# lucasjinreal/yolov7_d2

Hardware: AMD Instinct MI355X
Metric: images/sec training, YOLOX-s 640x640 bs=16/GPU (higher is better)
Workload: dtype bf16; 1 GPU; YOLOX-s CSPDarknet+PAFPN 640x640 bs=16/GPU: fwd + SimOTA loss + bwd + grad all-reduce + SGD(momentum) step, uint8 image batch + labels resident in HBM; global_batch=16, parallelism=dp1, hipgraph=True

## Files before the change

### yolov7_d2_amd/csrc/conv_igemm.hip

```cpp
#include <string.h>
#include <string.h>
#include "common.h"
#include "conv_igemm_kernel.h"
#include "conv1x1_stream.h"

bool c1s_try_launch(const mi_conv_desc* ds, int n, hipStream_t s, int* rc);
bool c1s_try_plan(const mi_conv_desc* ds, int n, C1Launch* l);
bool c1s_try_route(const mi_conv_desc* d);
int c1s_run_planned(const C1Launch* l, hipStream_t s);
bool c1s_try_plan_bn(const mi_conv_desc* ds, const mi_bn_job* bn, int n, C1Launch* l);
int c1s_barrier_status(unsigned* flag);
static_assert(sizeof(C1Launch) <= sizeof(((mi_conv_group*)0)->priv), "mi_conv_group.priv holds the stream launch record");
#include "conv3x3_ws.h"
bool w3_try_launch(const mi_conv_desc* ds, int n, hipStream_t s, int* rc);
bool w3_try_plan(const mi_conv_desc* ds, int n, W3Launch* l);
int w3_run_planned(const W3Launch* l, hipStream_t s);
bool w3_try_plan_bn(const mi_conv_desc* ds, const mi_bn_job* bn, int n, W3Launch* l);
int w3_barrier_status(unsigned* flag);
static_assert(sizeof(W3Launch) <= sizeof(((mi_conv_group*)0)->priv), "mi_conv_group.priv holds the 3x3 launch record");

#define MI_DECL_KC(KCv)                                                                      \
  int conv_launch_kc##KCv(const ConvK& k, int BN, int TPIX, size_t lds, hipStream_t s);       \
  int conv_group_launch_kc##KCv(const mi_conv_group* m, const ConvK* jobs, const int* starts, hipStream_t s);
MI_DECL_KC(16) MI_DECL_KC(32) MI_DECL_KC(64) MI_DECL_KC(128)
#undef MI_DECL_KC

static void choose_tile(int TPIX, int gridH, int gridW, int* TH, int* TW) {
  const int cands[] = {gridW, 64, 32, 16, 8, 4};
  long best = -1;
  int bh = 8, bw = 16;
  for (int c : cands) {
    if (c <= 0 || c > TPIX) continue;
    int tw = c;
    int th = TPIX / tw;
    if (th > gridH) th = gridH;
    if (th < 1) th = 1;
    long tiles = (long)mi_cdiv(gridH, th) * mi_cdiv(gridW, tw);
    long halo = (long)(th + 2) * (tw + 2);
    long score = tiles * 100000 + halo;
    if (best < 0 || score < best) {
      best = score;
      bh = th;
      bw = tw;
    }
  }
  *TH = bh;
  *TW = bw;
}

struct ConvCfg {
  int KC, BN, TPIX, TPS;
};

#ifdef MI_CONV_TIMELINE
static long long* g_conv_tl = nullptr;
extern "C" void mi_debug_conv_timeline(long long* dev_buf) { g_conv_tl = dev_buf; }
#endif
static int conv_fill(const mi_conv_desc* d, ConvK* k, ConvCfg* c, size_t* ldsBytes) {
  MI_REQUIRE(d->x && d->w && d->y, "conv: null pointer");
  MI_REQUIRE(d->ntaps >= 1 && d->ntaps <= MI_MAX_TAPS, "conv: ntaps %d", d->ntaps);
  MI_REQUIRE(d->K8 >= 2 && (d->K8 % 2) == 0, "conv: K8 %d must be even", d->K8);
  MI_REQUIRE(d->CoutPad % 32 == 0 && d->Cout <= d->CoutPad && d->Cout > 0, "conv: Cout %d pad %d",
             d->Cout, d->CoutPad);
  MI_REQUIRE(d->ldx % 8 == 0 && ((uintptr_t)d->x % 16) == 0, "conv: x must be 16B aligned (ldx %d)", d->ldx);
  MI_REQUIRE(d->in_stride == 1 || d->in_stride == 2, "conv: in_stride");
  MI_REQUIRE(d->out_stride == 1 || d->out_stride == 2, "conv: out_stride");
  MI_REQUIRE((long long)d->H * d->W * d->ldx < (1LL << 30), "conv: image plane too large for 32-bit offsets");
  if (!(d->flags & MI_CONV_OUT_F32))
    MI_REQUIRE((d->Cout % 4 != 0) || (d->ldy % 4 == 0 && ((uintptr_t)d->y % 8) == 0),
               "conv: bf16 y needs 8B alignment (ldy %d)", d->ldy);
  k->x = (const __bf16*)d->x;
  k->w = (const u32x4*)d->w;
  k->y = d->y;
  k->bias = d->bias;
  k->stats = d->stats_acc;
  k->nslots = (d->stats_slots >= 1 && d->stats_slots <= MI_BN_SLOTS) ? d->stats_slots : MI_BN_SLOTS;
  k->ynstride = d->y_nstride > 0 ? (long long)d->y_nstride : (long long)d->outH * d->outW * d->ldy;
  k->ldx = d->ldx; k->ldy = d->ldy; k->N = d->N; k->H = d->H; k->W = d->W;
  k->outH = d->outH; k->outW = d->outW; k->gridH = d->gridH; k->gridW = d->gridW;
  k->is = d->in_stride; k->os = d->out_stride; k->ooy = d->out_oy; k->oox = d->out_ox;
  k->K8 = d->K8; k->Cout = d->Cout; k->CoutPad = d->CoutPad; k->ntaps = d->ntaps;
  int dymin = 1 << 30, dymax = -(1 << 30), dxmin = 1 << 30, dxmax = -(1 << 30);
  for (int t = 0; t < d->ntaps; ++t) {
    k->tw[t] = d->tap_w[t];
    if (d->tap_dy[t] < dymin) dymin = d->tap_dy[t];
    if (d->tap_dy[t] > dymax) dymax = d->tap_dy[t];
    if (d->tap_dx[t] < dxmin) dxmin = d->tap_dx[t];
    if (d->tap_dx[t] > dxmax) dxmax = d->tap_dx[t];
  }
  k->flags = d->flags;
  {
    static const int noatom = getenv("MI_DEBUG_NOATOM") ? atoi(getenv("MI_DEBUG_NOATOM")) : 0;
    if (noatom) k->flags |= 1024;
  }
  MI_REQUIRE(!(d->flags & MI_CONV_RELU) || !((d->flags & (MI_CONV_ACCUM | MI_CONV_BNBWD | MI_CONV_OUT_F32 | MI_CONV_RELUMASK | MI_CONV_ADDRELU)) || d->stats_acc),
             "conv: MI_CONV_RELU is a plain forward epilogue (bf16 output, no accumulate / statistics)");
  if (d->flags & MI_CONV_BNBWD) {
    MI_REQUIRE(d->stats_acc && d->bn_y && d->bn_scale && d->bn_shift && d->bn_mean && d->bn_invstd,
               "conv: MI_CONV_BNBWD needs stats_acc and the producing layer's bn_* arrays");
    MI_REQUIRE(!(d->flags & MI_CONV_OUT_F32) && d->Cout % 8 == 0 && d->bn_ldy % 8 == 0 && ((uintptr_t)d->bn_y % 16) == 0,
               "conv: MI_CONV_BNBWD needs a bf16 output with Cout %% 8 == 0 (staged epilogue) and 16B-aligned bn_y");
    k->bn_y = (const __bf16*)d->bn_y; k->bn_scale = d->bn_scale; k->bn_shift = d->bn_shift;
    k->bn_mean = d->bn_mean; k->bn_invstd = d->bn_invstd; k->bn_ldy = d->bn_ldy; k->bn_act = d->bn_act;
  } else if (d->flags & (MI_CONV_RELUMASK | MI_CONV_ADDRELU)) {
    MI_REQUIRE((d->flags & (MI_CONV_RELUMASK | MI_CONV_ADDRELU)) != (MI_CONV_RELUMASK | MI_CONV_ADDRELU) && !d->stats_acc,
               "conv: MI_CONV_RELUMASK and MI_CONV_ADDRELU exclude each other and the forward statistics");
    MI_REQUIRE(d->bn_y && !(d->flags & MI_CONV_OUT_F32) && d->Cout % 8 == 0 && d->bn_ldy % 8 == 0 && d->bn_ldy >= d->Cout &&
               ((uintptr_t)d->bn_y % 16) == 0,
               "conv: the aux-tensor epilogue needs bn_y (16B-aligned, bn_ldy %% 8 == 0) and a bf16 output with Cout %% 8 == 0");
    k->bn_y = (const __bf16*)d->bn_y; k->bn_ldy = d->bn_ldy;
    k->bn_scale = k->bn_shift = k->bn_mean = k->bn_invstd = nullptr; k->bn_act = 0;
  } else {
    k->bn_y = nullptr; k->bn_scale = k->bn_shift = k->bn_mean = k->bn_invstd = nullptr; k->bn_ldy = 0; k->bn_act = 0;
  }
  const int Kp = d->K8 * 8;
  int BNmax = (d->CoutPad % 128 == 0) ? 128 : (d->CoutPad % 64 == 0) ? 64 : 32;
  int BN = d->BN, TPIX = 0, TH = d->TH, TW = d->TW;
  if (TH > 0 && TW > 0) TPIX = (TH * TW <= 64) ? 64 : 128;
  if (BN <= 0 || TPIX == 0) {
    const long want = 256;
    const int order[5][2] = {{128, 128}, {128, 64}, {64, 128}, {64, 64}, {64, 32}};
    int bestBN = BNmax, bestTP = TPIX ? TPIX : 128;
    for (int o = 0; o < 5; ++o) {
      const int tp = order[o][0];
      int bn = order[o][1];
      if (bn > BNmax) bn = BNmax;
      if (TPIX && tp != TPIX) continue;
      if (d->BN > 0 && bn != d->BN) continue;
      int th, tw;
      choose_tile(tp, d->gridH, d->gridW, &th, &tw);
      const long tiles = (long)d->N * mi_cdiv(d->gridH, th) * mi_cdiv(d->gridW, tw);
      bestBN = bn; bestTP = tp;
      if (tiles * (d->CoutPad / bn) >= want) break;
    }
    BN = bestBN; TPIX = bestTP;
  }
  MI_REQUIRE(BN == 32 || BN == 64 || BN == 128, "conv: BN %d", BN);
  MI_REQUIRE(d->CoutPad % BN == 0, "conv: CoutPad %d %% BN %d", d->CoutPad, BN);
  if (TH <= 0 || TW <= 0) choose_tile(TPIX, d->gridH, d->gridW, &TH, &TW);
  MI_REQUIRE(TH * TW <= TPIX && TH >= 1 && TW >= 1, "conv: tile %dx%d", TH, TW);
  k->TH = TH; k->TW = TW;
  k->tilesY = mi_cdiv(d->gridH, TH); k->tilesX = mi_cdiv(d->gridW, TW);
  k->dymin = dymin; k->dxmin = dxmin;
  const int haloH = (TH - 1) * d->in_stride + (dymax - dymin) + 1;
  k->haloW = (TW - 1) * d->in_stride + (dxmax - dxmin) + 1;
  k->npixh = haloH * k->haloW;
  for (int t = 0; t < d->ntaps; ++t) k->toff[t] = (d->tap_dy[t] - dymin) * k->haloW + (d->tap_dx[t] - dxmin);
  k->nco = d->CoutPad / BN;
  const long nblocks = (long)d->N * k->tilesY * k->tilesX * k->nco;
  int KC = d->KC, tps = d->TPS;
  auto lds_need = [&](int kc, int tp) {
    const size_t xb = (size_t)mi_cdiv(k->npixh, 64 / (kc / 8)) * 1024;
    const size_t wb = (size_t)tp * (kc / 8) * BN * 16;
    const int nch = Kp / kc, nst = nch * (d->ntaps / tp);
    return xb * (nch > 1 ? 2 : 1) + wb * (nst > 1 ? 2 : 1);
  };
  if (KC <= 0 || tps <= 0) {
    static const int maxkc = getenv("MI_CONV_MAXKC") ? atoi(getenv("MI_CONV_MAXKC")) : 128;
    static const int cap2 = getenv("MI_CONV_LDSCAP") ? atoi(getenv("MI_CONV_LDSCAP")) : 80;
    static const int cap1 = getenv("MI_CONV_LDSCAP1") ? atoi(getenv("MI_CONV_LDSCAP1")) : 160;
    static const double cS = getenv("MI_CONV_S") ? atof(getenv("MI_CONV_S")) : 0.25;
    static const double cT = getenv("MI_CONV_T") ? atof(getenv("MI_CONV_T")) : 0.3;
    static const int useocc = getenv("MI_CONV_OCC") ? atoi(getenv("MI_CONV_OCC")) : 1;
    const size_t cap = (size_t)(nblocks > 256 ? cap2 : cap1) * 1024;
    double bestCost = -1.0;
    int bk = 16, bt = 1;
    size_t bestLds = 0;
    const double vocc = BN == 32 ? 8.0 : (BN == 64 ? (TPIX == 128 ? 4.0 : 8.0) : (TPIX == 128 ? 3.0 : 5.0));
    const double gocc = nblocks > 256 ? nblocks / 256.0 : 1.0;
    const int kcs[4] = {128, 64, 32, 16};
    for (int ci = 0; ci < 4; ++ci) {
      const int kc = kcs[ci];
      if (Kp % kc != 0 || (d->KC > 0 && kc != d->KC) || (d->KC <= 0 && kc > maxkc)) continue;
      for (int tp = d->ntaps; tp >= 1; --tp) {
        if (d->ntaps % tp != 0 || (d->TPS > 0 && tp != d->TPS)) continue;
        const size_t need = lds_need(kc, tp);
        if (need > cap && !(kc == 16 && tp == 1)) continue;
        double occ = (double)((160 * 1024) / (need > 20480 ? need : 20480));
        if (occ < 1.0) occ = 1.0;
        if (occ > vocc) occ = vocc;
        if (occ > gocc) occ = gocc;
        if (!useocc) occ = 1.0;
        const double steps = (double)(Kp / kc) * (d->ntaps / tp), iters = (double)(Kp / kc) * d->ntaps;
        const double cost = (steps * cS + iters * cT) / occ;
        if (bestCost < 0 || cost < bestCost * 0.999 || (cost <= bestCost * 1.001 && need < bestLds)) {
          bestCost = cost; bk = kc; bt = tp; bestLds = need;
        }
      }
    }
    KC = bk; tps = bt;
  }
  MI_REQUIRE((KC == 16 || KC == 32 || KC == 64 || KC == 128) && Kp % KC == 0, "conv: KC %d for K %d", KC, Kp);
  MI_REQUIRE(tps >= 1 && d->ntaps % tps == 0, "conv: TPS %d for %d taps", tps, d->ntaps);
  const int RPI = 64 / (KC / 8);
  k->nqx = mi_cdiv(k->npixh, RPI);
  k->xbytes = k->nqx * 1024;
  MI_REQUIRE((long)k->nqx * RPI * k->haloW < (1 << 20) && k->nqx * RPI < 4096, "conv: halo too large for the row decode");
  k->mTW = ((1u << 20) + TW - 1) / TW;
  k->mHW = ((1u << 20) + k->haloW - 1) / k->haloW;
  const int nch = Kp / KC, nst = nch * (d->ntaps / tps);
  k->tps = tps;
  k->xstride = nch > 1 ? k->xbytes : 0;
  k->wstride = nst > 1 ? tps * (KC / 8) * BN * 16 : 0;
  c->KC = KC; c->BN = BN; c->TPIX = TPIX; c->TPS = tps;
  {
    static const int xm = getenv("MI_CONV_XMAP") ? atoi(getenv("MI_CONV_XMAP")) : 2;
    const bool on = xm >= 3 || (xm == 2 && (k->nco > 1 || d->ntaps > 1)) || (xm == 1 && k->nco > 1);
    k->xmap = (on && nblocks % 8 == 0) ? (int)(nblocks / 8) : 0;
#ifdef MI_CONV_TIMELINE
    k->tl = g_conv_tl;
#endif
  }
  *ldsBytes = lds_need(KC, tps);
  const size_t stage = (size_t)TPIX * (BN * 2 + 16);
  const size_t red = (size_t)16 * BN * 8;
  if (*ldsBytes < stage) *ldsBytes = stage;
  if (*ldsBytes < red) *ldsBytes = red;
  if (*ldsBytes < 4 * BN * 8) *ldsBytes = 4 * BN * 8;
  MI_REQUIRE(*ldsBytes <= 160 * 1024, "conv: LDS %zu too large", *ldsBytes);
  return MI_OK;
}

extern "C" int mi_conv2d_route(const mi_conv_desc* d) {
  MI_REQUIRE(d, "conv2d_route: null");
  if (c1s_try_route(d)) return 1;
  W3Launch wl;
  if (w3_try_plan(d, 1, &wl)) return 2;
  return d->xf ? -1 : 0;
}

extern "C" int mi_conv2d_plan(mi_conv_desc* d) {
  ConvK k;
  ConvCfg c;
  size_t lds;
  int rc = conv_fill(d, &k, &c, &lds);
  if (rc) return rc;
  d->TH = k.TH; d->TW = k.TW; d->KC = c.KC; d->BN = c.BN; d->TPS = c.TPS;
  return d->N * k.tilesY * k.tilesX;
}

extern "C" int mi_conv2d(const mi_conv_desc* d, mi_stream_t st) {
  {
    int rc = MI_OK;
    if (d && c1s_try_launch(d, 1, (hipStream_t)st, &rc)) return rc;
    if (d && w3_try_launch(d, 1, (hipStream_t)st, &rc)) return rc;
  }
  MI_REQUIRE(!d || !d->xf, "conv: the BatchNorm of the input (xf) runs on the streaming 1x1 / weight-stationary 3x3 kernels only");
  ConvK k;
  ConvCfg c;
  size_t lds;
  int rc = conv_fill(d, &k, &c, &lds);
  if (rc) return rc;
  hipStream_t s = (hipStream_t)st;
  static const long w8max = getenv("MI_CONV_W8") ? atol(getenv("MI_CONV_W8")) : (1L << 40);
  static const int w8mask = getenv("MI_CONV_W8MASK") ? atoi(getenv("MI_CONV_W8MASK")) : 7;
  const long nblocks = (long)k.N * k.tilesY * k.tilesX * k.nco;
  int tp = c.TPIX;
  const int cls = (c.TPIX == 128 && c.BN == 64) ? 1 : (c.TPIX == 128 && c.BN == 128) ? 2 : (c.TPIX == 64 && c.BN == 128) ? 4 : 0;
  if (nblocks <= w8max && (cls & w8mask) && !(d->flags & MI_CONV_OUT_F32) && (d->Cout & 7) == 0) {
    tp |= 1024;
  }
  switch (c.KC) {
    case 16: return conv_launch_kc16(k, c.BN, tp, lds, s);
    case 32: return conv_launch_kc32(k, c.BN, tp, lds, s);
    case 64: return conv_launch_kc64(k, c.BN, tp, lds, s);
    case 128: return conv_launch_kc128(k, c.BN, tp, lds, s);
  }
  MI_FAIL(MI_EINVAL, "conv: no kernel for KC %d BN %d TPIX %d", c.KC, c.BN, c.TPIX);
}

extern "C" int mi_conv2d_group_plan(const mi_conv_desc* descs, int n, void* table_host, int64_t table_cap,
                                    mi_conv_group* meta) {
  MI_REQUIRE(descs && meta && n >= 1 && n <= MI_CONV_MAX_GROUP, "conv_group_plan: 1..%d jobs", MI_CONV_MAX_GROUP);
  {
    C1Launch cl;
    if (c1s_try_plan(descs, n, &cl)) {
      memset(meta, 0, sizeof(*meta));
      meta->njobs = n; meta->nblocks = cl.grid; meta->lds_bytes = cl.lds;
      meta->KC = -1; meta->BN = cl.WM * 32; meta->TPIX = cl.PT; meta->TPS = cl.NBUF; meta->EPI = cl.MODE;
      meta->starts_off = 0; meta->table_bytes = 16;
      memcpy(meta->priv, &cl, sizeof(cl));
      if (table_host) {
        MI_REQUIRE(table_cap >= meta->table_bytes, "conv_group_plan: table too small");
        memset(table_host, 0, (size_t)meta->table_bytes);
      }
      return MI_OK;
    }
    W3Launch wl;
    if (w3_try_plan(descs, n, &wl)) {
      memset(meta, 0, sizeof(*meta));
      meta->njobs = n; meta->nblocks = wl.grid; meta->lds_bytes = wl.lds;
      meta->KC = -2; meta->BN = wl.K; meta->TPIX = 128; meta->TPS = 9; meta->EPI = wl.MODE;
      meta->starts_off = 0; meta->table_bytes = 16;
      memcpy(meta->priv, &wl, sizeof(wl));
      if (table_host) {
        MI_REQUIRE(table_cap >= meta->table_bytes, "conv_group_plan: table too small");
        memset(table_host, 0, (size_t)meta->table_bytes);
      }
      return MI_OK;
    }
  }
  for (int j = 0; j < n; ++j)
    MI_REQUIRE(!descs[j].xf, "conv_group_plan: the BatchNorm of the input (xf) runs on the streaming 1x1 / weight-stationary 3x3 kernels only");
  int big = 0;
  for (int j = 1; j < n; ++j)
    if ((long)descs[j].N * descs[j].gridH * descs[j].gridW > (long)descs[big].N * descs[big].gridH * descs[big].gridW) big = j;
  ConvK kb;
  ConvCfg cb;
  size_t lb;
  int rc = conv_fill(&descs[big], &kb, &cb, &lb);
  if (rc) return rc;
  ConvK ks[MI_CONV_MAX_GROUP];
  int starts[MI_CONV_MAX_GROUP + 1];
  size_t lds = 0;
  int epi = -1;
  starts[0] = 0;
  for (int j = 0; j < n; ++j) {
    mi_conv_desc d = descs[j];
    MI_REQUIRE((d.K8 * 8) % cb.KC == 0 && d.CoutPad % cb.BN == 0 && d.ntaps % cb.TPS == 0,
               "conv_group_plan: job %d does not fit the group's configuration (KC %d BN %d TPS %d)", j, cb.KC, cb.BN, cb.TPS);
    d.KC = cb.KC; d.BN = cb.BN; d.TPS = cb.TPS;
    ConvCfg c;
    size_t l = 0;
    if (j == big) {
      d.TH = kb.TH; d.TW = kb.TW;
      rc = conv_fill(&d, &ks[j], &c, &l);
      if (rc) return rc;
    } else {
      const size_t cap = lb > 80 * 1024 ? lb : 80 * 1024;
      const int cands[6][2] = {{0, 0}, {8, 16}, {4, 32}, {16, 8}, {8, 8}, {4, 16}};
      long bestTiles = -1;
      for (int q = 0; q < 6; ++q) {
        mi_conv_desc t = d;
        if (q == 0) {
          int th, tw;
          choose_tile(cb.TPIX, d.gridH, d.gridW, &th, &tw);
          t.TH = th; t.TW = tw;
        } else {
          t.TH = cands[q][0]; t.TW = cands[q][1];
        }
        if ((t.TH * t.TW <= 64 ? 64 : 128) != cb.TPIX) continue;
        ConvK kt;
        ConvCfg ct;
        size_t lt;
        if (conv_fill(&t, &kt, &ct, &lt) != MI_OK) continue;
        if (lt > cap || ct.KC != cb.KC || ct.BN != cb.BN || ct.TPS != cb.TPS) continue;
        const long tiles = (long)kt.N * kt.tilesY * kt.tilesX;
        if (bestTiles < 0 || tiles < bestTiles) { bestTiles = tiles; ks[j] = kt; c = ct; l = lt; }
      }
      MI_REQUIRE(bestTiles > 0, "conv_group_plan: job %d has no tile shape within the group's LDS footprint", j);
    }
    MI_REQUIRE(c.KC == cb.KC && c.BN == cb.BN && c.TPIX == cb.TPIX && c.TPS == cb.TPS,
               "conv_group_plan: job %d resolved to another configuration", j);
    MI_REQUIRE(!(ks[j].flags & (MI_CONV_RELUMASK | MI_CONV_ADDRELU)), "conv_group_plan: the aux-tensor epilogue (RELUMASK / ADDRELU) is a single-launch feature");
    const int e = (ks[j].flags & (MI_CONV_ACCUM | MI_CONV_BNBWD)) != 0;
    MI_REQUIRE(epi < 0 || epi == e, "conv_group_plan: jobs mix accumulating and plain launches");
    epi = e;
    if (l > lds) lds = l;
    if (starts[j] % 8) ks[j].xmap = 0;
    starts[j + 1] = starts[j] + ks[j].N * ks[j].tilesY * ks[j].tilesX * ks[j].nco;
  }
  int tpix = cb.TPIX;
  {
    static const long w8max = getenv("MI_CONV_W8G") ? atol(getenv("MI_CONV_W8G")) : (1L << 40);
    static const int w8mask = getenv("MI_CONV_W8MASK") ? atoi(getenv("MI_CONV_W8MASK")) : 7;
    const int cls = (cb.TPIX == 128 && cb.BN == 64) ? 1 : (cb.TPIX == 128 && cb.BN == 128) ? 2 : (cb.TPIX == 64 && cb.BN == 128) ? 4 : 0;
    bool staged = true;
    for (int j = 0; j < n; ++j) staged = staged && !(descs[j].flags & MI_CONV_OUT_F32) && (descs[j].Cout & 7) == 0;
    if (starts[n] <= w8max && (cls & w8mask) && staged) {
      tpix |= 1024;
    }
  }
  meta->njobs = n; meta->nblocks = starts[n]; meta->lds_bytes = (int32_t)lds;
  meta->KC = cb.KC; meta->BN = cb.BN; meta->TPIX = tpix; meta->TPS = cb.TPS; meta->EPI = epi;
  meta->starts_off = (int64_t)sizeof(ConvK) * n;
  meta->table_bytes = meta->starts_off + (int64_t)sizeof(int) * (n + 1);
  if (table_host) {
    MI_REQUIRE(table_cap >= meta->table_bytes, "conv_group_plan: table too small");
    memcpy(table_host, ks, sizeof(ConvK) * n);
    memcpy((char*)table_host + meta->starts_off, starts, sizeof(int) * (n + 1));
  }
  return MI_OK;
}

extern "C" int mi_conv2d_bn_plan(const mi_conv_desc* descs, const mi_bn_job* bn, int n, mi_conv_group* meta) {
  MI_REQUIRE(descs && bn && meta && n >= 1 && n <= MI_CONV_MAX_GROUP, "conv_bn_plan: 1..%d jobs", MI_CONV_MAX_GROUP);
  C1Launch cl;
  if (c1s_try_plan_bn(descs, bn, n, &cl)) {
    memset(meta, 0, sizeof(*meta));
    meta->njobs = n; meta->nblocks = cl.grid; meta->lds_bytes = cl.lds;
    meta->KC = -1; meta->BN = cl.WM * 32; meta->TPIX = cl.PT; meta->TPS = cl.NBUF; meta->EPI = cl.MODE;
    meta->table_bytes = 16;
    memcpy(meta->priv, &cl, sizeof(cl));
    return 1;
  }
  W3Launch wl;
  if (w3_try_plan_bn(descs, bn, n, &wl)) {
    memset(meta, 0, sizeof(*meta));
    meta->njobs = n; meta->nblocks = wl.grid; meta->lds_bytes = wl.lds;
    meta->KC = -2; meta->BN = wl.K; meta->TPIX = 128; meta->TPS = 9; meta->EPI = wl.MODE;
    meta->table_bytes = 16;
    memcpy(meta->priv, &wl, sizeof(wl));
    return 1;
  }
  return 0;
}

extern "C" int mi_conv2d_bn_fwd(const mi_conv_desc* descs, const mi_bn_job* bn, int n, mi_stream_t st) {
  mi_conv_group meta;
  const int rc = mi_conv2d_bn_plan(descs, bn, n, &meta);
  if (rc < 0) return rc;
  MI_REQUIRE(rc == 1, "conv_bn_fwd: needs convolutions that run on the streaming 1x1 (at most %d of one input) or the weight-"
             "stationary 3x3 kernel with stats_acc, each followed by the train-mode BatchNorm of exactly its output", C1_MAX_BN);
  if (meta.KC == -1) return c1s_run_planned((const C1Launch*)meta.priv, (hipStream_t)st);
  return w3_run_planned((const W3Launch*)meta.priv, (hipStream_t)st);
}

extern "C" int mi_conv_bn_barrier_status(uint32_t* flags) {
  MI_REQUIRE(flags, "conv_bn_barrier_status: null");
  unsigned a = 0, b = 0;
  int rc = c1s_barrier_status(&a);
  if (rc) return rc;
  rc = w3_barrier_status(&b);
  if (rc) return rc;
  *flags = (a ? 1u : 0u) | (b ? 2u : 0u);
  return MI_OK;
}

extern "C" int mi_conv2d_group_run(const mi_conv_group* m, const void* table_dev, mi_stream_t st) {
  MI_REQUIRE(m && (table_dev || m->KC < 0) && m->njobs >= 1, "conv_group_run: null");
  if (m->KC == -1) return c1s_run_planned((const C1Launch*)m->priv, (hipStream_t)st);
  if (m->KC == -2) return w3_run_planned((const W3Launch*)m->priv, (hipStream_t)st);
  const ConvK* jobs = (const ConvK*)table_dev;
  const int* starts = (const int*)((const char*)table_dev + m->starts_off);
  hipStream_t s = (hipStream_t)st;
  switch (m->KC) {
    case 16: return conv_group_launch_kc16(m, jobs, starts, s);
    case 32: return conv_group_launch_kc32(m, jobs, starts, s);
    case 64: return conv_group_launch_kc64(m, jobs, starts, s);
    case 128: return conv_group_launch_kc128(m, jobs, starts, s);
  }
  MI_FAIL(MI_EINVAL, "conv_group: no kernel for KC %d BN %d TPIX %d", m->KC, m->BN, m->TPIX);
}

__device__ __forceinline__ void pack_w_body(const float* __restrict__ w, int Cout, int Cin, int KK, __bf16* wf,
                                            int CinPad, int CoutPad, __bf16* wd, int CoutPadK, int CinPadN,
                                            const float* __restrict__ cs = nullptr) {
  const int64_t nf = wf ? (int64_t)KK * CinPad * CoutPad : 0;
  const int64_t nd = wd ? (int64_t)KK * CoutPadK * CinPadN : 0;
  for (int64_t idx = blockIdx.x * (int64_t)blockDim.x + threadIdx.x; idx < nf + nd;
       idx += (int64_t)gridDim.x * blockDim.x) {
    if (idx < nf) {
      const int e = idx & 7;
      int64_t r = idx >> 3;
      const int co = r % CoutPad; r /= CoutPad;
      const int k8 = r % (CinPad / 8);
      const int tap = r / (CinPad / 8);
      const int ci = k8 * 8 + e;
      float v = 0.f;
      if (co < Cout && ci < Cin) v = w[((int64_t)co * Cin + ci) * KK + tap] * (cs ? cs[co] : 1.f);
      wf[idx] = (__bf16)v;
    } else {
      const int64_t i2 = idx - nf;
      const int e = i2 & 7;
      int64_t r = i2 >> 3;
      const int ci = r % CinPadN; r /= CinPadN;
      const int k8 = r % (CoutPadK / 8);
      const int tap = r / (CoutPadK / 8);
      const int co = k8 * 8 + e;
      float v = 0.f;
      if (co < Cout && ci < Cin) v = w[((int64_t)co * Cin + ci) * KK + tap] * (cs ? cs[co] : 1.f);
      wd[i2] = (__bf16)v;
    }
  }
}

__global__ void pack_w_kernel(const float* __restrict__ w, int Cout, int Cin, int KK, __bf16* wf, int CinPad,
                              int CoutPad, __bf16* wd, int CoutPadK, int CinPadN) {
  pack_w_body(w, Cout, Cin, KK, wf, CinPad, CoutPad, wd, CoutPadK, CinPadN);
}
__global__ void pack_w_scaled_kernel(const float* __restrict__ w, const float* __restrict__ cs, int Cout, int Cin, int KK,
                                     __bf16* wf, int CinPad, int CoutPad, __bf16* wd, int CoutPadK, int CinPadN) {
  pack_w_body(w, Cout, Cin, KK, wf, CinPad, CoutPad, wd, CoutPadK, CinPadN, cs);
}
#define PK_CO 32
#define PK_CI 64
__global__ __launch_bounds__(256) void pack_w_batch_kernel(const mi_pack_job* __restrict__ jobs, int njobs, int kk_max) {
  extern __shared__ __attribute__((aligned(16))) __bf16 pk_s[];
  int lo = 0, hi = njobs - 1;
  while (lo < hi) {
    const int mid = (lo + hi + 1) >> 1;
    if (jobs[mid].blk0 <= (int)blockIdx.x) lo = mid; else hi = mid - 1;
  }
  const mi_pack_job j = jobs[lo];
  const int KK = j.KK, tid = threadIdx.x;
  const int coP = j.wd && j.CoutPadK > j.CoutPad ? j.CoutPadK : (j.wf ? j.CoutPad : j.CoutPadK);
  const int nco_t = (coP + PK_CO - 1) / PK_CO;
  const int t = (int)blockIdx.x - j.blk0;
  const int co0 = (t % nco_t) * PK_CO, ci0 = (t / nco_t) * PK_CI;
  const int rs = PK_CI * kk_max + 2;
  int nci = j.Cin - ci0;
  nci = nci < 0 ? 0 : (nci > PK_CI ? PK_CI : nci);
  const int rowlen = PK_CI * KK;
  const float* const wrow0 = j.w + ((size_t)co0 * j.Cin + ci0) * KK;
  const bool fast = nci == PK_CI && co0 + PK_CO <= j.Cout && ((j.Cin * KK) & 3) == 0 && (((uintptr_t)wrow0) & 15) == 0 &&
                    (rowlen & 3) == 0;
  if (fast) {
    const int wave = tid >> 6, lane = tid & 63;
    for (int co_l = wave; co_l < PK_CO; co_l += 4) {
      const float4* src = (const float4*)(wrow0 + (size_t)co_l * j.Cin * KK);
      const float sc = j.scale ? j.scale[co0 + co_l] : 1.f;
      unsigned* dst = (unsigned*)(pk_s + co_l * rs);
      for (int q4 = lane; q4 < rowlen / 4; q4 += 64) {
        const float4 v = src[q4];
        const __bf16 b0 = (__bf16)(v.x * sc), b1 = (__bf16)(v.y * sc), b2 = (__bf16)(v.z * sc), b3 = (__bf16)(v.w * sc);
        dst[2 * q4] = (unsigned)__builtin_bit_cast(unsigned short, b0) | ((unsigned)__builtin_bit_cast(unsigned short, b1) << 16);
        dst[2 * q4 + 1] = (unsigned)__builtin_bit_cast(unsigned short, b2) | ((unsigned)__builtin_bit_cast(unsigned short, b3) << 16);
      }
    }
  } else
  for (int idx = tid; idx < PK_CO * rowlen; idx += 256) {
    const int co_l = idx / rowlen, q = idx - co_l * rowlen;
    const int row = co0 + co_l;
    float v = 0.f;
    if (row < j.Cout && q < nci * KK) {
      v = j.w[((size_t)row * j.Cin + ci0) * KK + q];
      if (j.scale) v *= j.scale[row];
    }
    pk_s[co_l * rs + q] = (__bf16)v;
  }
  __syncthreads();
  const int K8f = j.CinPad / 8, K8d = j.CoutPadK / 8;
  if (j.wf) {
    for (int it = tid; it < KK * 256; it += 256) {
      const int tap = it >> 8, k8_l = (it >> 5) & 7, co_l = it & 31;
      const int k8 = ci0 / 8 + k8_l, co = co0 + co_l;
      if (k8 >= K8f || co >= j.CoutPad) continue;
      unsigned short h[8];
#pragma unroll
      for (int e = 0; e < 8; ++e) h[e] = __builtin_bit_cast(unsigned short, pk_s[co_l * rs + (k8_l * 8 + e) * KK + tap]);
      ((uint4*)j.wf)[((size_t)tap * K8f + k8) * j.CoutPad + co] =
          make_uint4(h[0] | ((uint32_t)h[1] << 16), h[2] | ((uint32_t)h[3] << 16), h[4] | ((uint32_t)h[5] << 16),
                     h[6] | ((uint32_t)h[7] << 16));
    }
  }
  if (j.wd) {
    for (int it = tid; it < KK * 256; it += 256) {
      const int tap = it >> 8, co8_l = (it >> 6) & 3, ci_l = it & 63;
      const int co8 = co0 / 8 + co8_l, ci = ci0 + ci_l;
      if (co8 >= K8d || ci >= j.CinPadN) continue;
      unsigned short h[8];
#pragma unroll
      for (int e = 0; e < 8; ++e) h[e] = __builtin_bit_cast(unsigned short, pk_s[(co8_l * 8 + e) * rs + ci_l * KK + tap]);
      ((uint4*)j.wd)[((size_t)tap * K8d + co8) * j.CinPadN + ci] =
          make_uint4(h[0] | ((uint32_t)h[1] << 16), h[2] | ((uint32_t)h[3] << 16), h[4] | ((uint32_t)h[5] << 16),
                     h[6] | ((uint32_t)h[7] << 16));
    }
  }
}
static int pack_tiles(const mi_pack_job& j) {
  const int coP = j.wd && j.CoutPadK > j.CoutPad ? j.CoutPadK : (j.wf ? j.CoutPad : j.CoutPadK);
  const int ciP = j.wd && j.CinPadN > j.CinPad ? j.CinPadN : (j.wf ? j.CinPad : j.CinPadN);
  return ((coP + PK_CO - 1) / PK_CO) * ((ciP + PK_CI - 1) / PK_CI);
}
extern "C" int mi_pack_jobs_layout(mi_pack_job* jobs_host, int njobs) {
  MI_REQUIRE(jobs_host && njobs > 0, "pack_jobs_layout: args");
  int64_t blk = 0;
  for (int k = 0; k < njobs; ++k) {
    mi_pack_job& j = jobs_host[k];
    MI_REQUIRE(j.w && (j.wf || j.wd) && j.KK >= 1 && j.KK <= MI_MAX_TAPS, "pack_jobs_layout: job %d: null / taps", k);
    if (j.wf) MI_REQUIRE(j.CinPad % 8 == 0 && j.CinPad >= j.Cin && j.CoutPad >= j.Cout, "pack_jobs_layout: job %d: fwd pads", k);
    if (j.wd) MI_REQUIRE(j.CoutPadK % 8 == 0 && j.CoutPadK >= j.Cout && j.CinPadN >= j.Cin, "pack_jobs_layout: job %d: dgrad pads", k);
    j.blk0 = (int32_t)blk;
    blk += pack_tiles(j);
    MI_REQUIRE(blk < (1LL << 30), "pack_jobs_layout: too many blocks");
  }
  return (int)blk;
}
extern "C" int mi_pack_conv_weights_batch(const mi_pack_job* jobs_dev, int njobs, int total_blocks, int kk_max,
                                          mi_stream_t st) {
  MI_REQUIRE(jobs_dev && njobs > 0 && total_blocks > 0 && kk_max >= 1 && kk_max <= MI_MAX_TAPS, "pack_w_batch: args");
  const size_t lds = (size_t)PK_CO * (PK_CI * kk_max + 2) * 2;
  static bool attr_done = false;
  if (!attr_done) {
    hipFuncSetAttribute((const void*)pack_w_batch_kernel, hipFuncAttributeMaxDynamicSharedMemorySize, 80 * 1024);
    attr_done = true;
  }
  hipLaunchKernelGGL(pack_w_batch_kernel, dim3(total_blocks), dim3(256), lds, (hipStream_t)st, jobs_dev, njobs, kk_max);
  MI_CHECK_LAUNCH("pack_w_batch");
  return MI_OK;
}

extern "C" int mi_pack_conv_weight(const float* w, int Cout, int Cin, int KH, int KW, void* wf, int CinPad,
                                   int CoutPad, void* wd, int CoutPadK, int CinPadN, mi_stream_t st) {
  MI_REQUIRE(w && (wf || wd), "pack_w: null");
  if (wf) MI_REQUIRE(CinPad % 8 == 0 && CinPad >= Cin && CoutPad >= Cout, "pack_w: fwd pads");
  if (wd) MI_REQUIRE(CoutPadK % 8 == 0 && CoutPadK >= Cout && CinPadN >= Cin, "pack_w: dgrad pads");
  const int KK = KH * KW;
  const int64_t n = (wf ? (int64_t)KK * CinPad * CoutPad : 0) + (wd ? (int64_t)KK * CoutPadK * CinPadN : 0);
  int blocks = (int)((n + 255) / 256);
  if (blocks > 2048) blocks = 2048;
  hipLaunchKernelGGL(pack_w_kernel, dim3(blocks), dim3(256), 0, (hipStream_t)st, w, Cout, Cin, KK, (__bf16*)wf,
                     CinPad, CoutPad, (__bf16*)wd, CoutPadK, CinPadN);
  MI_CHECK_LAUNCH("pack_w");
  return MI_OK;
}

extern "C" int mi_pack_conv_weight_scaled(const float* w, const float* cout_scale, int Cout, int Cin, int KH, int KW, void* wf, int CinPad,
                                   int CoutPad, void* wd, int CoutPadK, int CinPadN, mi_stream_t st) {
  MI_REQUIRE(w && cout_scale && (wf || wd), "pack_w_scaled: null");
  if (wf) MI_REQUIRE(CinPad % 8 == 0 && CinPad >= Cin && CoutPad >= Cout, "pack_w: fwd pads");
  if (wd) MI_REQUIRE(CoutPadK % 8 == 0 && CoutPadK >= Cout && CinPadN >= Cin, "pack_w: dgrad pads");
  const int KK = KH * KW;
  const int64_t n = (wf ? (int64_t)KK * CinPad * CoutPad : 0) + (wd ? (int64_t)KK * CoutPadK * CinPadN : 0);
  int blocks = (int)((n + 255) / 256);
  if (blocks > 2048) blocks = 2048;
  hipLaunchKernelGGL(pack_w_scaled_kernel, dim3(blocks), dim3(256), 0, (hipStream_t)st, w, cout_scale, Cout, Cin, KK, (__bf16*)wf,
                     CinPad, CoutPad, (__bf16*)wd, CoutPadK, CinPadN);
  MI_CHECK_LAUNCH("pack_w_scaled");
  return MI_OK;
}
```

Baseline: 3062 images/sec.

## Add weight-stationary fused kernel for stride-2 3x3 conv data gradient

Adds a dedicated kernel for the data gradient of stride-2 3x3 convolutions. It handles all four output parity classes in one persistent launch, keeps the 9 weight taps resident in registers, and double-buffers input tiles into LDS with async loads. The generic grouped implicit-GEMM path previously ran this as four parity sub-convolutions. The new kernel aims to cut weight reloads and launch/tile overhead and to reuse the staged input across classes. In exchange it adds significant code complexity, high register pressure (occupancy 1-2), and a narrow eligibility check that falls back to the old path otherwise.

```diff
diff --git a/yolov7_d2_amd/csrc/conv_dgrad2_ws.h b/yolov7_d2_amd/csrc/conv_dgrad2_ws.h
--- /dev/null
+++ b/yolov7_d2_amd/csrc/conv_dgrad2_ws.h
@@ -0,0 +1,240 @@
+#pragma once
+#include <type_traits>
+#include "conv3x3_ws.h"
+
+#define DG2_MAX_JOBS 8
+#define DG2_TH 8
+#define DG2_HW 17
+
+struct DG2Job {
+  const __bf16* x;
+  const u32x4* w;
+  __bf16* y;
+  int ldx, ldy, N, H, W;
+  int inH, inW;
+  int tilesY, tilesX, ntiles;
+  int blk0, nblk, wld;
+  int tw[9];
+};
+struct DG2K {
+  int njobs, pad_;
+  DG2Job j[DG2_MAX_JOBS];
+};
+struct DG2Launch {
+  int K, WM, ACC, grid, lds, pad_;
+  DG2K k;
+};
+
+constexpr int dg2_ntap(int p) { return p ? 2 : 1; }
+constexpr int dg2_wpos(int p, int t) { return p ? (t == 0 ? 0 : 2) : 1; }
+constexpr int dg2_off(int p, int t) { return p ? (t == 0 ? 1 : 0) : 0; }
+
+template <int K, int WM, int ACC>
+__global__ __launch_bounds__(256, K == 128 ? 1 : 2) void conv_igemm_dgrad2_ws_kernel(const DG2K p) {
+  constexpr int NW = 4, WN = NW / WM, G = WM, KC8 = K / 8, KS = K / 16;
+  constexpr int HW = DG2_HW, HPIX = (DG2_TH + 1) * HW, HROWS = (HPIX + 63) / 64 * 64;
+  static_assert(WN * G * 32 == DG2_TH * W3_TW, "pixel tile");
+  constexpr int PLANE = HROWS * 16;
+  constexpr int NQ = (HROWS / 64) * KC8;
+  constexpr int D = NQ / NW;
+  static_assert(NQ % NW == 0 && D >= 1, "DMA split");
+  constexpr int XB = KC8 * PLANE;
+  static_assert((KC8 - 1) * PLANE + (HW + 1) * 16 < 65536, "ds_read immediate");
+  constexpr int NST = 2 * G;
+
+  extern __shared__ __attribute__((aligned(16))) char smem[];
+  const unsigned lds0 = (unsigned)(uintptr_t)(__attribute__((address_space(3))) char*)smem;
+  const int tid = threadIdx.x, lane = tid & 63;
+  const int wave = __builtin_amdgcn_readfirstlane(tid >> 6);
+  const int wm = wave / WN, wn = wave % WN;
+  const int l31 = lane & 31, h = lane >> 5;
+
+  int ji = 0;
+  while (ji + 1 < p.njobs && (int)blockIdx.x >= p.j[ji + 1].blk0) ++ji;
+  ji = __builtin_amdgcn_readfirstlane(ji);
+  const DG2Job& jb = p.j[ji];
+  const int b = (int)blockIdx.x - jb.blk0, nb = jb.nblk;
+  const int nt = (jb.ntiles - b + nb - 1) / nb;
+  const int H = jb.H, Wd = jb.W, inH = jb.inH, inW = jb.inW, tilesX = jb.tilesX, tpi = jb.tilesY * jb.tilesX;
+  const int ldxb = jb.ldx * 2, ldyb = jb.ldy * 2;
+  const char* const xbase = (const char*)jb.x;
+  char* const ybase = (char*)jb.y;
+  const char* zpage = (const char*)g_w3_zero_page;
+  asm volatile("" : "+s"(zpage));
+
+  bf16x8 a[9][KS];
+  {
+    const u32x4* wb = jb.w + wm * 32 + l31;
+#pragma unroll
+    for (int t = 0; t < 9; ++t) {
+      const int slab = jb.tw[t] * KC8;
+#pragma unroll
+      for (int ks = 0; ks < KS; ++ks) a[t][ks] = __builtin_bit_cast(bf16x8, wb[(size_t)(slab + ks * 2 + h) * jb.wld]);
+    }
+  }
+
+  struct Org { int img, i0, j0; };
+  auto tile_origin = [&](int i) {
+    const int t = b + i * nb;
+    Org o;
+    o.img = t / tpi;
+    const int rem = t - o.img * tpi, tyq = rem / tilesX;
+    o.i0 = tyq * DG2_TH;
+    o.j0 = (rem - tyq * tilesX) * W3_TW;
+    return o;
+  };
+  auto issue_x1 = [&](const Org& o, int buf, int d) {
+    const char* xt = xbase + ((size_t)o.img * inH * inW + (size_t)o.i0 * inW + o.j0) * (size_t)ldxb;
+    const int q = wave * D + d;
+    const int pb = q / KC8, k8 = q % KC8;
+    const unsigned pix = (unsigned)(pb * 64 + lane);
+    const int hy = (int)(pix / (unsigned)HW);
+    const int hx = (int)pix - hy * HW;
+    const bool v = ((int)pix < HPIX) & (o.i0 + hy < inH) & (o.j0 + hx < inW);
+    const char* g = v ? xt + (unsigned)((hy * inW + hx) * ldxb + k8 * 16) : zpage;
+    w3_glds16(g, lds0 + buf * XB + k8 * PLANE + pb * 1024);
+  };
+
+  int lg, lidx;
+  {
+    const int l = l31;
+    lg = ((l >= 4) & (l < 12)) | ((l >= 16) & (l < 20)) | (l >= 28);
+    lidx = l - (l < 4 ? 0 : l < 12 ? 4 : l < 20 ? 8 : l < 28 ? 12 : 16);
+  }
+  unsigned bbase[G];
+#pragma unroll
+  for (int g = 0; g < G; ++g) bbase[g] = (unsigned)(h * PLANE + (((wn * G + g) * 2 + lg) * HW + lidx) * 16);
+  auto out_ptr = [&](const Org& o, int g, int py, int px) -> char* {
+    const int oy = 2 * (o.i0 + (wn * G + g) * 2 + lg) + py, ox = 2 * (o.j0 + lidx) + px;
+    char* q = ybase + (((size_t)o.img * H + oy) * Wd + ox) * (size_t)ldyb + wm * 64 + h * 16;
+    return ((oy < H) & (ox < Wd)) ? q : nullptr;
+  };
+
+  Org oc = tile_origin(0), op = oc;
+#pragma unroll
+  for (int d = 0; d < D; ++d) issue_x1(oc, 0, d);
+
+  u32x4 pk[NST];
+  auto store_deferred = [&]() {
+#pragma unroll
+    for (int l = 0; l < NST; ++l) {
+      char* q = out_ptr(op, l / 2, 0, 0);
+      if (q) *(u32x4*)(q + (l % 2) * 32) = pk[l];
+    }
+  };
+  for (int i = 0; i < nt; ++i) {
+    W3_VMCNT(0);
+    __builtin_amdgcn_s_barrier();
+    const bool more = i + 1 < nt;
+    const Org on = tile_origin(more ? i + 1 : i);
+    const char* Xs = smem + (i & 1) * XB;
+    if (more) {
+#pragma unroll
+      for (int d = 0; d < D; ++d) issue_x1(on, (i + 1) & 1, d);
+    }
+    if (i > 0) store_deferred();
+
+    auto do_class = [&](auto PYc, auto PXc) {
+      constexpr int py = decltype(PYc)::value, px = decltype(PXc)::value, cls = py * 2 + px;
+      constexpr int NTX = dg2_ntap(px), NS = dg2_ntap(py) * NTX * KS;
+      u32x4 old[NST];
+      if constexpr (ACC) {
+#pragma unroll
+        for (int l = 0; l < NST; ++l) {
+          const char* q = out_ptr(oc, l / 2, py, px);
+          old[l] = q ? *(const u32x4*)(q + (l % 2) * 32) : u32x4{0u, 0u, 0u, 0u};
+        }
+      }
+      f32x16 acc[G];
+#pragma unroll
+      for (int g = 0; g < G; ++g)
+#pragma unroll
+        for (int r = 0; r < 16; ++r) acc[g][r] = 0.f;
+      auto ldb = [&](int step, bf16x8(&dst)[G]) {
+        const int t = step / KS, ks = step % KS, ty = t / NTX, tx = t % NTX;
+        const int off = (dg2_off(py, ty) * HW + dg2_off(px, tx)) * 16 + 2 * ks * PLANE;
+#pragma unroll
+        for (int g = 0; g < G; ++g) dst[g] = __builtin_bit_cast(bf16x8, *(const u32x4*)(Xs + bbase[g] + off));
+      };
+      bf16x8 bf[3][G];
+      ldb(0, bf[0]);
+      ldb(1, bf[1]);
+#pragma unroll
+      for (int st = 0; st < NS; ++st) {
+        __builtin_amdgcn_sched_barrier(0);
+        if (st + 2 < NS) ldb(st + 2, bf[(st + 2) % 3]);
+        const int t = st / KS, wpos = dg2_wpos(py, t / NTX) * 3 + dg2_wpos(px, t % NTX);
+#pragma unroll
+        for (int g = 0; g < G; ++g)
+          acc[g] = __builtin_amdgcn_mfma_f32_32x32x16_bf16(a[wpos][st % KS], bf[st % 3][g], acc[g], 0, 0, 0);
+#pragma unroll
+        for (int g = 0; g < G; ++g) {
+          __builtin_amdgcn_sched_group_barrier(0x008, 1, 0);
+          __builtin_amdgcn_sched_group_barrier(0x100, 1, 0);
+        }
+      }
+      __builtin_amdgcn_sched_barrier(0);
+
+#pragma unroll
+      for (int g = 0; g < G; ++g) {
+        unsigned pw[8];
+#pragma unroll
+        for (int q = 0; q < 4; ++q) {
+          bf16x4 o;
+#pragma unroll
+          for (int e = 0; e < 4; ++e) o[e] = (__bf16)acc[g][4 * q + e];
+          const u32x2 u = __builtin_bit_cast(u32x2, o);
+          pw[2 * q] = u[0];
+          pw[2 * q + 1] = u[1];
+        }
+        char* const q = out_ptr(oc, g, py, px);
+#pragma unroll
+        for (int pr = 0; pr < 2; ++pr) {
+          const int q0 = 2 * pr, q1 = 2 * pr + 1;
+          const auto w0 = __builtin_amdgcn_permlane32_swap(pw[2 * q0], pw[2 * q1], false, false);
+          const auto w1 = __builtin_amdgcn_permlane32_swap(pw[2 * q0 + 1], pw[2 * q1 + 1], false, false);
+          u32x4 v = {w0[0], w1[0], w0[1], w1[1]};
+          if constexpr (ACC) {
+            const bf16x8 nv = __builtin_bit_cast(bf16x8, v), ov = __builtin_bit_cast(bf16x8, old[g * 2 + pr]);
+            bf16x8 rv;
+#pragma unroll
+            for (int e = 0; e < 8; ++e) rv[e] = (__bf16)((float)nv[e] + (float)ov[e]);
+            v = __builtin_bit_cast(u32x4, rv);
+          }
+          if constexpr (cls == 0) pk[g * 2 + pr] = v;
+          else if (q) *(u32x4*)(q + pr * 32) = v;
+        }
+      }
+    };
+    do_class(std::integral_constant<int, 1>{}, std::integral_constant<int, 1>{});
+    do_class(std::integral_constant<int, 1>{}, std::integral_constant<int, 0>{});
+    do_class(std::integral_constant<int, 0>{}, std::integral_constant<int, 1>{});
+    do_class(std::integral_constant<int, 0>{}, std::integral_constant<int, 0>{});
+    op = oc;
+    oc = on;
+  }
+  store_deferred();
+}
+
+template <int K, int WM, int ACC>
+static int dg2_launch_one(const DG2Launch& l, hipStream_t s) {
+  auto fn = conv_igemm_dgrad2_ws_kernel<K, WM, ACC>;
+  static bool attr_done = false;
+  if (!attr_done) {
+    hipFuncSetAttribute((const void*)fn, hipFuncAttributeMaxDynamicSharedMemorySize, 160 * 1024);
+    attr_done = true;
+  }
+  hipLaunchKernelGGL(fn, dim3((unsigned)l.grid), dim3(256), (size_t)l.lds, s, l.k);
+  MI_CHECK_LAUNCH("conv_dgrad2_ws");
+  return MI_OK;
+}
+constexpr int dg2_max_block_cout(int K) { return K == 128 ? 128 : 32; }
+template <int K>
+static int dg2_launch_k(const DG2Launch& l, hipStream_t s) {
+  if (l.WM == 1) return l.ACC ? dg2_launch_one<K, 1, 1>(l, s) : dg2_launch_one<K, 1, 0>(l, s);
+  if constexpr (dg2_max_block_cout(K) == 128) {
+    if (l.WM == 2) return l.ACC ? dg2_launch_one<K, 2, 1>(l, s) : dg2_launch_one<K, 2, 0>(l, s);
+    if (l.WM == 4) return l.ACC ? dg2_launch_one<K, 4, 1>(l, s) : dg2_launch_one<K, 4, 0>(l, s);
+  }
+  MI_FAIL(MI_EINVAL, "conv_dgrad2_ws: K %d with %d dx channels per block", K, l.WM * 32);
+}
diff --git a/yolov7_d2_amd/csrc/conv_dgrad2_ws.hip b/yolov7_d2_amd/csrc/conv_dgrad2_ws.hip
--- /dev/null
+++ b/yolov7_d2_amd/csrc/conv_dgrad2_ws.hip
@@ -0,0 +1,98 @@
+#include <stdlib.h>
+#include <string.h>
+#include "common.h"
+#include "conv_dgrad2_ws.h"
+
+int dg2_launch_k64(const DG2Launch& l, hipStream_t s);
+int dg2_launch_k128(const DG2Launch& l, hipStream_t s);
+
+static int dg2_cus() {
+  static int cus = 0;
+  if (!cus) {
+    int dev = 0;
+    hipDeviceProp_t pr;
+    if (hipGetDevice(&dev) == hipSuccess && hipGetDeviceProperties(&pr, dev) == hipSuccess) cus = pr.multiProcessorCount;
+    if (cus <= 0) cus = 256;
+  }
+  return cus;
+}
+
+static bool dg2_enabled() {
+  const char* ws = getenv("MI_CONV_WS");
+  const char* e = getenv("MI_CONV_WS_DG2");
+  return (!ws || atoi(ws) != 0) && (!e || atoi(e) != 0);
+}
+
+bool dg2_try_plan(const mi_conv_desc* ds, int n, DG2Launch* l) {
+  if (n != 4 || !dg2_enabled()) return false;
+  const mi_conv_desc& d0 = ds[0];
+  const int K = d0.K8 * 8;
+  if (K != 64 && K != 128) return false;
+  if (d0.flags & ~MI_CONV_ACCUM) return false;
+  if (d0.Cout != d0.CoutPad || d0.Cout % 32) return false;
+  const int bc = d0.Cout <= dg2_max_block_cout(K) ? d0.Cout : dg2_max_block_cout(K);
+  if ((bc != 32 && bc != 64 && bc != 128) || d0.Cout % bc || d0.Cout / bc > DG2_MAX_JOBS) return false;
+  if (d0.N < 1 || d0.outH < 1 || d0.outW < 1) return false;
+  if (d0.H != (d0.outH - 1) / 2 + 1 || d0.W != (d0.outW - 1) / 2 + 1) return false;
+  if (d0.ldx % 8 || d0.ldy % 8 || ((uintptr_t)d0.x & 15) || ((uintptr_t)d0.y & 15) || ((uintptr_t)d0.w & 15)) return false;
+  if (!d0.x || !d0.y || !d0.w || d0.ldx < K || d0.ldy < d0.Cout) return false;
+  if (d0.y_nstride && (long long)d0.y_nstride != (long long)d0.outH * d0.outW * d0.ldy) return false;
+  if ((long long)d0.H * d0.W * d0.ldx * 2 >= (1LL << 31) || (long long)d0.outH * d0.outW * d0.ldy * 2 >= (1LL << 31)) return false;
+  int tw[9], seen_cls = 0, seen_pos = 0, seen_slab = 0;
+  for (int j = 0; j < 4; ++j) {
+    const mi_conv_desc& d = ds[j];
+    if (d.bias || d.stats_acc || d.xf || d.bn_y || d.flags != d0.flags) return false;
+    if (d.x != d0.x || d.w != d0.w || d.y != d0.y || d.ldx != d0.ldx || d.ldy != d0.ldy || d.y_nstride != d0.y_nstride) return false;
+    if (d.N != d0.N || d.H != d0.H || d.W != d0.W || d.outH != d0.outH || d.outW != d0.outW) return false;
+    if (d.K8 != d0.K8 || d.Cout != d0.Cout || d.CoutPad != d0.CoutPad) return false;
+    if (d.in_stride != 1 || d.out_stride != 2) return false;
+    const int py = d.out_oy, px = d.out_ox;
+    if ((py & ~1) || (px & ~1) || (seen_cls & (1 << (py * 2 + px)))) return false;
+    seen_cls |= 1 << (py * 2 + px);
+    if (d.gridH != (d.outH - py + 1) / 2 || d.gridW != (d.outW - px + 1) / 2) return false;
+    if (d.ntaps != dg2_ntap(py) * dg2_ntap(px)) return false;
+    for (int t = 0; t < d.ntaps; ++t) {
+      const int oy = d.tap_dy[t], ox = d.tap_dx[t], s = d.tap_w[t];
+      if ((oy & ~1) || (ox & ~1) || (!py && oy) || (!px && ox) || s < 0 || s > 8) return false;
+      const int pos = (py ? (oy ? 0 : 2) : 1) * 3 + (px ? (ox ? 0 : 2) : 1);
+      if ((seen_pos & (1 << pos)) || (seen_slab & (1 << s))) return false;
+      seen_pos |= 1 << pos;
+      seen_slab |= 1 << s;
+      tw[pos] = s;
+    }
+  }
+  if (seen_cls != 0xf || seen_pos != 0x1ff || seen_slab != 0x1ff) return false;
+
+  memset(l, 0, sizeof(*l));
+  const int nj = d0.Cout / bc;
+  const int tilesY = mi_cdiv(d0.H, DG2_TH), tilesX = mi_cdiv(d0.W, W3_TW);
+  const long long ntiles = (long long)d0.N * tilesY * tilesX;
+  if (ntiles >= (1LL << 30)) return false;
+  long long per_job = (long long)dg2_cus() * (K == 128 ? 1 : 2) / nj;
+  if (per_job < 1) per_job = 1;
+  if (per_job > ntiles) per_job = ntiles;
+  for (int j = 0; j < nj; ++j) {
+    DG2Job& jb = l->k.j[j];
+    memcpy(jb.tw, tw, sizeof(tw));
+    jb.x = (const __bf16*)d0.x; jb.w = (const u32x4*)d0.w + j * bc; jb.y = (__bf16*)d0.y + j * bc;
+    jb.ldx = d0.ldx; jb.ldy = d0.ldy; jb.N = d0.N; jb.H = d0.outH; jb.W = d0.outW; jb.inH = d0.H; jb.inW = d0.W;
+    jb.tilesY = tilesY; jb.tilesX = tilesX; jb.ntiles = (int)ntiles;
+    jb.wld = d0.CoutPad;
+    jb.blk0 = j * (int)per_job; jb.nblk = (int)per_job;
+  }
+  l->k.njobs = nj;
+  l->K = K;
+  l->WM = bc / 32;
+  l->ACC = (d0.flags & MI_CONV_ACCUM) ? 1 : 0;
+  l->grid = nj * (int)per_job;
+  l->lds = 2 * (K / 8) * (((DG2_TH + 1) * DG2_HW + 63) / 64 * 64) * 16;
+  return true;
+}
+
+int dg2_run_planned(const DG2Launch* l, hipStream_t s) {
+  switch (l->K) {
+    case 64: return dg2_launch_k64(*l, s);
+    case 128: return dg2_launch_k128(*l, s);
+  }
+  MI_FAIL(MI_EINVAL, "conv_dgrad2_ws: K %d", l->K);
+}
diff --git a/yolov7_d2_amd/csrc/conv_dgrad2_ws_k128.hip b/yolov7_d2_amd/csrc/conv_dgrad2_ws_k128.hip
--- /dev/null
+++ b/yolov7_d2_amd/csrc/conv_dgrad2_ws_k128.hip
@@ -0,0 +1,2 @@
+#include "conv_dgrad2_ws.h"
+int dg2_launch_k128(const DG2Launch& l, hipStream_t s) { return dg2_launch_k<128>(l, s); }
diff --git a/yolov7_d2_amd/csrc/conv_dgrad2_ws_k64.hip b/yolov7_d2_amd/csrc/conv_dgrad2_ws_k64.hip
--- /dev/null
+++ b/yolov7_d2_amd/csrc/conv_dgrad2_ws_k64.hip
@@ -0,0 +1,2 @@
+#include "conv_dgrad2_ws.h"
+int dg2_launch_k64(const DG2Launch& l, hipStream_t s) { return dg2_launch_k<64>(l, s); }
diff --git a/yolov7_d2_amd/csrc/conv_igemm.hip b/yolov7_d2_amd/csrc/conv_igemm.hip
--- a/yolov7_d2_amd/csrc/conv_igemm.hip
+++ b/yolov7_d2_amd/csrc/conv_igemm.hip
@@ -18,6 +18,10 @@
 bool w3_try_plan_bn(const mi_conv_desc* ds, const mi_bn_job* bn, int n, W3Launch* l);
 int w3_barrier_status(unsigned* flag);
 static_assert(sizeof(W3Launch) <= sizeof(((mi_conv_group*)0)->priv), "mi_conv_group.priv holds the 3x3 launch record");
+#include "conv_dgrad2_ws.h"
+bool dg2_try_plan(const mi_conv_desc* ds, int n, DG2Launch* l);
+int dg2_run_planned(const DG2Launch* l, hipStream_t s);
+static_assert(sizeof(DG2Launch) <= sizeof(((mi_conv_group*)0)->priv), "mi_conv_group.priv holds the stride-2 data-gradient launch record");
 
 #define MI_DECL_KC(KCv)                                                                      \
   int conv_launch_kc##KCv(const ConvK& k, int BN, int TPIX, size_t lds, hipStream_t s);       \
@@ -299,6 +303,19 @@
       }
       return MI_OK;
     }
+    DG2Launch dl;
+    if (dg2_try_plan(descs, n, &dl)) {
+      memset(meta, 0, sizeof(*meta));
+      meta->njobs = n; meta->nblocks = dl.grid; meta->lds_bytes = dl.lds;
+      meta->KC = -3; meta->BN = dl.WM * 32; meta->TPIX = 128; meta->TPS = 9; meta->EPI = dl.ACC;
+      meta->starts_off = 0; meta->table_bytes = 16;
+      memcpy(meta->priv, &dl, sizeof(dl));
+      if (table_host) {
+        MI_REQUIRE(table_cap >= meta->table_bytes, "conv_group_plan: table too small");
+        memset(table_host, 0, (size_t)meta->table_bytes);
+      }
+      return MI_OK;
+    }
   }
   for (int j = 0; j < n; ++j)
     MI_REQUIRE(!descs[j].xf, "conv_group_plan: the BatchNorm of the input (xf) runs on the streaming 1x1 / weight-stationary 3x3 kernels only");
@@ -431,6 +448,7 @@
   MI_REQUIRE(m && (table_dev || m->KC < 0) && m->njobs >= 1, "conv_group_run: null");
   if (m->KC == -1) return c1s_run_planned((const C1Launch*)m->priv, (hipStream_t)st);
   if (m->KC == -2) return w3_run_planned((const W3Launch*)m->priv, (hipStream_t)st);
+  if (m->KC == -3) return dg2_run_planned((const DG2Launch*)m->priv, (hipStream_t)st);
   const ConvK* jobs = (const ConvK*)table_dev;
   const int* starts = (const int*)((const char*)table_dev + m->starts_off);
   hipStream_t s = (hipStream_t)st;
```

Result: no change. 3091 images/sec (median of 6 runs) (+1.0%).
